# triq-org/spectroplot-js

Hardware: NVIDIA B200
Metric: Msamples/s rendered to RGBA spectrogram (N=4096) and % of B200 HBM roofline (higher is better)
Workload: dtype f32

## Files before the change

spectroplot-js_b200/csrc/sp_kernel_r64.cuh:

```cuda
#pragma once
#include "sp_prims.cuh"

#ifndef SP_XP
#define SP_XP 0
#endif
#ifndef SP_R64_TMA
#define SP_R64_TMA 1
#endif

namespace sp {

template <int FMT, bool SUB> struct R64Cfg {
    static constexpr int N = 4096, T = 64, STREAMS = 4, FFT_THREADS = T * STREAMS, STORE_THREADS = 128, THREADS = FFT_THREADS + STORE_THREADS;
    static constexpr int STEPS = 4, F = STREAMS * STEPS;
    static constexpr int FFT_REGS = 232, STORE_REGS = 40;
    static constexpr int SWB = SUB ? 8 : sample_width(FMT == FMT_RUNTIME ? CF64 : FMT);
    static constexpr bool OK = SUB || ((FMT != FMT_RUNTIME) && SWB <= 8);
    static constexpr int XP = 66;
    static constexpr int X_BYTES = 64 * XP * 8;
    static constexpr int WIN_PITCH = 64;
    static constexpr int TW_PITCH = 14;
    static constexpr int ST_PITCH = 1026;
    static constexpr int RING = 4;
    static constexpr bool TMA = SP_R64_TMA != 0;
    static constexpr int TILE_BYTES = TMA ? (STORE_THREADS / 32) * 4096 : 0;
    static constexpr size_t SMEM_BYTES = (size_t)STREAMS * X_BYTES + (size_t)F * ST_PITCH * 4 + (size_t)JH_SIZE * 4
                                       + ((SUB || TMA) ? 0 : (size_t)T * WIN_PITCH * 4) + TILE_BYTES + (size_t)T * TW_PITCH * 8 + 1024
                                       + (size_t)F * 2 * 8  + (size_t)2 * F * 8  + 192 + 1024 ;
    static_assert(SMEM_BYTES <= 232448, "render_r64_kernel: dynamic shared memory above the 227 KB an sm_100 CTA may have");
};

__device__ __forceinline__ unsigned lut_at(unsigned lut_base, unsigned word, int j)
{
    const unsigned a = ((j == 0 ? word << 2 : word >> (8 * j - 2)) & 0x3fcu) | lut_base;
    unsigned v;
    asm volatile("ld.shared.u32 %0, [%1];" : "=r"(v) : "r"(a));
    return v;
}

__device__ __forceinline__ void store_row8(uint32_t *rowp, uint4 a, uint4 b, bool aligned)
{
    if (aligned) st_global_256(rowp, a, b);
    else {
        rowp[0] = a.x; rowp[1] = a.y; rowp[2] = a.z; rowp[3] = a.w;
        rowp[4] = b.x; rowp[5] = b.y; rowp[6] = b.z; rowp[7] = b.w;
    }
}

__device__ __forceinline__ void stream_barrier(int stream)
{
    asm volatile("bar.sync %0, 64;" ::"r"(stream + 1) : "memory");
}

template <int FMT, bool SUB, bool OPT = false>
__global__ void __launch_bounds__(384, 1) render_r64_kernel(const Params p, const float2 *__restrict__ tw14, const __grid_constant__ CUtensorMap tmap)
{
    using B = R64Cfg<FMT, SUB>;
    constexpr int N = B::N, T = B::T, F = B::F;
    constexpr bool FLOAT_IN = SUB || FMT == CF32 || FMT == CF64 || FMT == FMT_RUNTIME;
    extern __shared__ __align__(128) unsigned char smem_r64[];
    const unsigned lut_base = (smem_u32(smem_r64) + 1023u) & ~1023u;
    unsigned char *s_x = smem_r64 + (lut_base - smem_u32(smem_r64)) + 1024;
    unsigned *s_lut = reinterpret_cast<unsigned *>(s_x - 1024);
    unsigned char *s_tiles = s_x + B::STREAMS * B::X_BYTES;
    unsigned *s_stage = reinterpret_cast<unsigned *>(s_tiles + B::TILE_BYTES);
    unsigned *s_jh = s_stage + F * B::ST_PITCH;
    float *s_win = reinterpret_cast<float *>(s_jh + JH_SIZE);
    float2 *s_tw = reinterpret_cast<float2 *>(s_win + ((SUB || B::TMA) ? 0 : T * B::WIN_PITCH));
    uint2 *s_mm = reinterpret_cast<uint2 *>(s_tw + T * B::TW_PITCH);
    float2 *s_fmid = reinterpret_cast<float2 *>(s_mm + F * 2);
    uint64_t *s_mbar = reinterpret_cast<uint64_t *>(s_fmid + 2 * F);
    int *s_off = reinterpret_cast<int *>(s_mbar + B::STREAMS);
    uint64_t *s_full = reinterpret_cast<uint64_t *>(s_off + B::STREAMS * 2);
    uint64_t *s_empty = s_full + 2;
    uint64_t *s_tready = s_empty + 2;
    long long *s_ring = reinterpret_cast<long long *>(s_tready + B::RING);
    long long *s_tile0 = s_ring + B::RING;

    const int tid = threadIdx.x;
    const int s = tid >> 6;
    const int t = tid & 63;
    float2 *X = reinterpret_cast<float2 *>(s_x + (size_t)s * B::X_BYTES);
    unsigned char *raw = reinterpret_cast<unsigned char *>(X);
    uint64_t *mbar = s_mbar + s;

    for (int i = tid; i < JH_SIZE; i += B::THREADS) s_jh[i] = 0;
    const int cmax = p.cmap_len - 1;
    const JhConst jc = jh_const(p);
    for (int i = tid; i < 256; i += B::THREADS) s_lut[i] = i <= cmax ? p.lut[jc.rev ? cmax - i : i] : 0u;
    for (int i = tid; i < T * B::TW_PITCH; i += B::THREADS) s_tw[i] = tw14[i];
    if constexpr (!SUB && !B::TMA)
        for (int i = tid; i < N; i += B::THREADS) s_win[(i & 63) * B::WIN_PITCH + (((i >> 6) + 4 * (i & 63)) & 63)] = p.window[i];
    const unsigned jh_base = smem_u32(s_jh) - (JH_MAGIC_BITS << 2);
    const int nfull = p.n_full, sub_r = p.sub_r;

    auto stage = [&](long long xr, int k0sub, unsigned par) {
        if (xr >= p.chunk_frames) xr = p.chunk_frames - 1;
        const void *src;
        unsigned bytes;
        if constexpr (SUB) {
            src = p.sub_in + ((size_t)xr * sub_r + (size_t)k0sub) * N;
            bytes = N * 8;
            s_off[s * 2 + par] = 0;
        } else {
            const long long xgl = p.frame_first + p.chunk_first + xr;
            const long long p0 = (long long)__dadd_rn(0.5, __dmul_rn(p.stride, (double)xgl)) - p.sample_base;
            const unsigned long long off = (unsigned long long)p0 * B::SWB, a0 = off & ~15ull;
            src = p.buf + a0;
            bytes = (unsigned)(((off - a0) + (unsigned long long)N * B::SWB + 15) & ~15ull);
            s_off[s * 2 + par] = (int)(off - a0);
        }
        tma_load_1d(raw, src, bytes, mbar);
    };
    auto tile_xr0 = [&](long long tile) -> long long { return (SUB ? tile / sub_r : tile) * F; };

    auto ticket = [&]() -> long long {
        const unsigned long long k = atomicAdd(p.tile_ctr, 1ull);
        if (k == (unsigned long long)p.ntiles + gridDim.x - 1) atomicExch(p.tile_ctr, 0ull);
        return (long long)k;
    };
    auto ring_put = [&](unsigned j, long long tl) {
        s_ring[(j - 1) % B::RING] = tl;
        mbar_arrive(s_tready + (j - 1) % B::RING);
    };
    auto ring_get = [&](unsigned j) -> long long {
        mbar_wait(s_tready + (j - 1) % B::RING, ((j - 1) / B::RING) & 1);
        return s_ring[(j - 1) % B::RING];
    };

    if (p.t_stamp && blockIdx.x == 0 && tid == 0) p.t_stamp[0] = globaltimer_ns();
    if (t == 0 && tid < B::FFT_THREADS) mbar_init(mbar, 1);
    if (tid == 0) {
        for (int h = 0; h < 2; h++) { mbar_init(s_full + h, B::FFT_THREADS / 32); mbar_init(s_empty + h, B::STORE_THREADS / 32); }
        for (int r = 0; r < B::RING; r++) mbar_init(s_tready + r, 1);
    }
    if (tid == B::FFT_THREADS) *s_tile0 = ticket();
    if (t == 0) asm volatile("fence.mbarrier_init.release.cluster;" ::: "memory");
    __syncthreads();
    long long tile = *s_tile0;
    unsigned kk = 0;

    if (tid >= B::FFT_THREADS) {
        asm volatile("setmaxnreg.dec.sync.aligned.u32 %0;" ::"n"(B::STORE_REGS));
        const int ht = tid - B::FFT_THREADS;
        const bool rows_aligned = (p.nframes % 8 == 0) && ((reinterpret_cast<uintptr_t>(p.image) & 31) == 0);
        if (ht == 0 && tile < p.ntiles) ring_put(1, ticket());
        griddep_wait();
        griddep_launch_dependents();
        while (tile < p.ntiles) {
            const int k0sub = SUB ? (int)(tile % sub_r) : 0;
            const long long xr0 = tile_xr0(tile);
#pragma unroll 1
            for (int h = 0; h < 2; h++) {
                mbar_wait(s_full + h, kk & 1);
                const size_t x0 = (size_t)(p.chunk_first + xr0) + 8 * h;
                const bool live = xr0 + 8 * h < p.chunk_frames;
                if constexpr (OPT && !SUB) {
                    if (p.waterfall && live) {
#pragma unroll 1
                        for (int f = 0; f < 8; f++) {
                            uint32_t *rowp = reinterpret_cast<uint32_t *>(p.image) + (size_t)N * (size_t)(p.nframes - 1 - (long long)(x0 + f));
                            const unsigned *src = s_stage + (8 * h + f) * B::ST_PITCH + ht;
#pragma unroll
                            for (int i = 0; i < 8; i++) {
                                const int id = ht + B::STORE_THREADS * i, k0 = id & 63, m = id >> 6;
                                const unsigned w = src[B::STORE_THREADS * i];
#pragma unroll
                                for (int j = 0; j < 4; j++)
                                    rowp[(k0 + 64 * (4 * m + j) + N / 2 - 1) & (N - 1)] = lut_at(lut_base, w, j);
                            }
                        }
                    }
                }
                if constexpr (B::TMA && !SUB) {
                    if (p.use_tma && live && (!OPT || !p.waterfall)) {
                        const int lane = ht & 31, wq = ht >> 5;
                        unsigned char *tile = s_tiles + wq * 4096;
                        const int r = 31 - lane;
                        const unsigned toff = (unsigned)(r * 32 + (((r >> 2) & 1) << 4));
#pragma unroll 1
                        for (int i = 0; i < 8; i++) {
                            const int id = ht + B::STORE_THREADS * i, k0 = id & 63, m = id >> 6;
                            const unsigned *src = s_stage + (8 * h) * B::ST_PITCH + m * 64 + k0;
                            unsigned w[8];
#pragma unroll
                            for (int f = 0; f < 8; f++) w[f] = src[f * B::ST_PITCH];
                            if (lane == 0) bulk_wait_read0();
                            __syncwarp();
#pragma unroll
                            for (int j = 0; j < 4; j++) {
                                uint4 a, b;
                                a.x = lut_at(lut_base, w[0], j); a.y = lut_at(lut_base, w[1], j); a.z = lut_at(lut_base, w[2], j); a.w = lut_at(lut_base, w[3], j);
                                b.x = lut_at(lut_base, w[4], j); b.y = lut_at(lut_base, w[5], j); b.z = lut_at(lut_base, w[6], j); b.w = lut_at(lut_base, w[7], j);
                                *reinterpret_cast<uint4 *>(tile + j * 1024 + toff) = a;
                                *reinterpret_cast<uint4 *>(tile + j * 1024 + (toff ^ 16u)) = b;
                                if (k0 + 64 * (4 * m + j) == N / 2)
                                    st_global_256(reinterpret_cast<uint32_t *>(p.image) + x0, a, b);
                            }
                            fence_async_smem();
                            __syncwarp();
                            if (lane == 0) {
                                const int kb0 = (k0 & 32) + 256 * m;
#pragma unroll
                                for (int j = 0; j < 4; j++)
                                    tma_store_2d(&tmap, smem_u32(tile + j * 1024), (int)x0, (N / 2 - (kb0 + 64 * j) - 31) & (N - 1));
                                bulk_commit();
                            }
                        }
                    }
                }
#pragma unroll 1
                for (int i = 0; i < ((live && (!OPT || SUB || !p.waterfall) && !(B::TMA && !SUB && p.use_tma)) ? 8 : 0); i++) {
                    const int id = ht + B::STORE_THREADS * i, k0 = id & 63, m = id >> 6;
                    const unsigned *src = s_stage + (8 * h) * B::ST_PITCH + m * 64 + k0;
                    unsigned w[8];
#pragma unroll
                    for (int f = 0; f < 8; f++) w[f] = src[f * B::ST_PITCH];
#pragma unroll
                    for (int j = 0; j < 4; j++) {
                        const int kb = k0 + 64 * (4 * m + j);
                        const int bin = SUB ? k0sub + sub_r * kb : kb;
                        const int y = (nfull / 2 - bin) & (nfull - 1);
                        uint32_t *rowp = reinterpret_cast<uint32_t *>(p.image) + (size_t)p.nframes * (size_t)y + x0;
                        uint4 a, b;
                        if (!(p.dbg & 4)) {
                            a.x = lut_at(lut_base, w[0], j); a.y = lut_at(lut_base, w[1], j); a.z = lut_at(lut_base, w[2], j); a.w = lut_at(lut_base, w[3], j);
                            b.x = lut_at(lut_base, w[4], j); b.y = lut_at(lut_base, w[5], j); b.z = lut_at(lut_base, w[6], j); b.w = lut_at(lut_base, w[7], j);
                        } else { a = make_uint4(w[0], w[1], w[2], w[3]); b = make_uint4(w[4], w[5], w[6], w[7]); }
                        if (!(p.dbg & 1)) store_row8(rowp, a, b, rows_aligned);
                    }
                }
                if (ht < 8 && live) {
                    const int fl = 8 * h + ht;
                    const long long xl = p.chunk_first + xr0 + fl;
                    const uint2 m0 = s_mm[fl * 2], m1 = s_mm[fl * 2 + 1];
                    const unsigned umn = min(m0.x, m1.x), umx = max(m0.y, m1.y);
                    const float mn = fminf(0.0f, fmaf(fast_log2(__uint_as_float(umn)), p.c1, p.c0));
                    const float mx = fmaxf(-200.0f, fmaf(fast_log2(__uint_as_float(umx)), p.c1, p.c0));
                    if constexpr (SUB) {
                        atomicMin(reinterpret_cast<unsigned *>(p.fmin) + xl, f2ord(mn));
                        atomicMax(reinterpret_cast<unsigned *>(p.fmax) + xl, f2ord(mx));
                    } else { p.fmin[xl] = mn; p.fmax[xl] = mx; p.fmid[xl] = s_fmid[(kk & 1) * F + fl]; }
                }
                __syncwarp();
                if ((ht & 31) == 0) mbar_arrive(s_empty + h);
            }
            tile = ring_get(++kk);
            if (ht == 0 && tile < p.ntiles) ring_put(kk + 1, ticket());
        }
        if constexpr (B::TMA && !SUB) bulk_wait_read0();
    } else {
    asm volatile("setmaxnreg.inc.sync.aligned.u32 %0;" ::"n"(B::FFT_REGS));
    unsigned fpar = 0;
    if (t == 0 && tile < p.ntiles) stage(tile_xr0(tile) + s, SUB ? (int)(tile % sub_r) : 0, 0);

    while (tile < p.ntiles) {
        const int k0sub = SUB ? (int)(tile % sub_r) : 0;
        const long long xr0 = tile_xr0(tile);
        long long next_tile = 0;

#pragma unroll 1
        for (int step = 0; step < B::STEPS; step++) {
            const int fl = step * B::STREAMS + s;
            const bool valid = xr0 + fl < p.chunk_frames;
            const unsigned jbase = valid ? jh_base : jh_base + (smem_u32(s_stage + 8 * B::ST_PITCH) - smem_u32(s_jh));
            int half = step >> 1;
            asm volatile("" : "+r"(half));
            if (step == B::STEPS - 1) next_tile = ring_get(kk + 1);
            cf v[64];
            const bool split = OPT && !SUB && p.channel_mode;
            auto prefetch = [&]() {
                if (step < B::STEPS - 1) stage(xr0 + fl + B::STREAMS, k0sub, fpar);
                else if (next_tile < p.ntiles) stage(tile_xr0(next_tile) + s, SUB ? (int)(next_tile % sub_r) : 0, fpar);
            };
            mbar_wait(mbar, fpar);
            if constexpr (SUB) {
#pragma unroll
                for (int n0 = 0; n0 < 8; n0++)
#pragma unroll
                    for (int n1 = 0; n1 < 8; n1++) v[8 * n1 + n0] = cld(reinterpret_cast<const float2 *>(raw) + T * (8 * n1 + n0) + t);
            } else {
                const unsigned char *rp = raw + s_off[s * 2 + fpar];
                const float4 *wrow = B::TMA ? p.window_t + t : reinterpret_cast<const float4 *>(s_win + t * B::WIN_PITCH);
#pragma unroll
                for (int qq = 0; qq < 16; qq++) {
                    const int q = 2 * (qq & 7) + (qq >> 3);
                    const float4 w = (SP_XP & 4) ? make_float4(1.f, 1.f, 1.f, 1.f) : B::TMA ? __ldg(wrow + 64 * q) : wrow[(q + t) & 15];
                    cf d[4];
#pragma unroll
                    for (int c = 0; c < 4; c++) d[c] = decode_raw_cf<FMT>(rp, T * (4 * q + c) + t, p.format);
                    if (q == 8 && t == 0 && valid) s_fmid[(kk & 1) * F + fl] = make_float2(cre(d[0]) * raw_scale<FMT>(), cim(d[0]) * raw_scale<FMT>());
                    v[4 * q] = cscale(d[0], w.x);     v[4 * q + 1] = cscale(d[1], w.y);
                    v[4 * q + 2] = cscale(d[2], w.z); v[4 * q + 3] = cscale(d[3], w.w);
                }
            }
            fpar ^= 1;
            dft64_between(v, [&] { stream_barrier(s); });
            {
                const float4 *twp = reinterpret_cast<const float4 *>(s_tw + t * B::TW_PITCH);
                float2 w[8];
                const float4 a = twp[0], b = twp[1], c = twp[2], d = twp[3];
                w[1] = make_float2(a.x, a.y); w[2] = make_float2(a.z, a.w); w[3] = make_float2(b.x, b.y); w[4] = make_float2(b.z, b.w);
                w[5] = make_float2(c.x, c.y); w[6] = make_float2(c.z, c.w); w[7] = make_float2(d.x, d.y);
#pragma unroll
                for (int j = 1; j < 8; j++) v[j] = cmul(v[j], w[j]);
#pragma unroll
                for (int j = 0; j < 8; j++) cst(X + j * B::XP + t, v[j]);
                float2 hi[8];
                hi[1] = make_float2(d.z, d.w);
                const float4 e = twp[4], f = twp[5], g = twp[6];
                hi[2] = make_float2(e.x, e.y); hi[3] = make_float2(e.z, e.w); hi[4] = make_float2(f.x, f.y);
                hi[5] = make_float2(f.z, f.w); hi[6] = make_float2(g.x, g.y); hi[7] = make_float2(g.z, g.w);
#pragma unroll
                for (int i = 1; i < 8; i++) {
                    v[8 * i] = cmul(v[8 * i], hi[i]);
#pragma unroll
                    for (int j = 1; j < 8; j++) v[8 * i + j] = cmul(v[8 * i + j], (SP_XP & 8) ? w[j] : cun(cmul(cpk(hi[i]), w[j])));
#pragma unroll
                    for (int j = 0; j < 8; j++) cst(X + (8 * i + j) * B::XP + t, v[8 * i + j]);
                }
            }
            stream_barrier(s);
            {
                const float4 *row = reinterpret_cast<const float4 *>(X + t * B::XP);
#pragma unroll
                for (int mm = 0; mm < 32; mm++) {
                    const int m = 4 * (mm & 7) + (mm >> 3);
                    const float4 q = row[m];
                    v[2 * m] = cpk(q.x, q.y); v[2 * m + 1] = cpk(q.z, q.w);
                }
            }
            dft64_between(v, [&] {
                stream_barrier(s);
                if (t == 0 && !split) prefetch();
            });
            if ((step & 1) == 0) mbar_wait(s_empty + half, (kk + 1) & 1);
            {
                {
                    if constexpr (OPT && !SUB) {
                        if (split) {
                            auto split_lo = [](cf a, cf b) {
                                const float2 fb = cun(b);
                                return cscale(cadd(a, cpk(fb.x, -fb.y)), 0.5f);
                            };
                            auto split_hi = [](cf a, cf b) {
                                const float2 fa = cun(a), fb = cun(b);
                                return cscale(cadd(cpk(fa.y, fa.x), cpk(fb.y, -fb.x)), 0.5f);
                            };
                            {
                                float4 *wrow = reinterpret_cast<float4 *>(X + t * B::XP);
#pragma unroll
                                for (int m = 0; m < 32; m++) {
                                    const float2 a = cun(v[2 * m]), b = cun(v[2 * m + 1]);
                                    wrow[m] = make_float4(a.x, a.y, b.x, b.y);
                                }
                            }
                            stream_barrier(s);
                            if (t == 0) {
#pragma unroll
                                for (int k1 = 1; k1 < 32; k1++) {
                                    const cf a = v[k1], b = v[64 - k1];
                                    v[k1] = split_lo(a, b);
                                    v[64 - k1] = split_hi(b, a);
                                }
                                v[0] = cpk(fmaf(0.0f, cim(v[0]), cre(v[0])), 0.0f);
                                v[32] = cpk(0.0f, 0.0f);
                            } else {
                                const float4 *prow = reinterpret_cast<const float4 *>(X + (64 - t) * B::XP);
#pragma unroll
                                for (int a = 0; a < 32; a++) {
                                    const float4 q = prow[31 - a];
                                    if (a < 16) {
                                        v[2 * a] = split_lo(v[2 * a], cpk(q.z, q.w));
                                        v[2 * a + 1] = split_lo(v[2 * a + 1], cpk(q.x, q.y));
                                    } else {
                                        v[2 * a] = split_hi(v[2 * a], cpk(q.z, q.w));
                                        v[2 * a + 1] = split_hi(v[2 * a + 1], cpk(q.x, q.y));
                                    }
                                }
                            }
                            stream_barrier(s);
                            if (t == 0) prefetch();
                        }
                    }

                    float amin = __int_as_float(0x7f800000), amax = 0.0f, prev = 0.0f;
                    unsigned umin_i = 0x7f800000u, umax_i = 0u;
                    unsigned *stg = s_stage + fl * B::ST_PITCH + t;
#pragma unroll
                    for (int m = 0; m < 16; m++) {
                        unsigned yb[4];
#pragma unroll
                        for (int j = 0; j < 4; j++) {
                            const float2 vi = cun(v[4 * m + j]);
                            const float abs2 = fmaf(vi.x, vi.x, vi.y * vi.y);
                            if constexpr (FLOAT_IN) {
                                umin_i = min(umin_i, __float_as_uint(abs2));
                                umax_i = max(umax_i, __float_as_uint(abs2));
                            } else if (j & 1) {
                                amin = fmin3(amin, prev, abs2);
                                amax = fmax3(amax, prev, abs2);
                            } else prev = abs2;
                            const float l2 = (SP_XP & 16) ? abs2 : fast_log2(abs2);
                            float Y;
                            const float S = (SP_XP & 16) ? (Y = l2, __uint_as_float((__float_as_uint(l2) >> 20) + JH_MAGIC_BITS)) : jh_eval(l2, jc, Y);
                            if constexpr ((SP_XP & 1) != 0) red_shared_inc_addr(smem_u32(s_jh) + ((tid & 31) << 2) + (__float_as_uint(S) & 0x380u));
                            else if constexpr (!(SP_XP & 2)) red_shared_inc_addr(jbase + (__float_as_uint(S) << 2));
                            yb[j] = __float_as_uint(Y);
                        }
                        stg[m * 64] = __byte_perm(__byte_perm(yb[0], yb[1], 0x0040), __byte_perm(yb[2], yb[3], 0x0040), 0x5410);
                    }
                    unsigned umn, umx;
                    if constexpr (FLOAT_IN) {
                        umn = __reduce_min_sync(0xffffffffu, umin_i);
                        umx = __reduce_max_sync(0xffffffffu, umax_i);
                    } else {
                        umn = __reduce_min_sync(0xffffffffu, __float_as_uint(amin));
                        umx = __reduce_max_sync(0xffffffffu, __float_as_uint(amax));
                    }
                    if (umn < 0x00800000u || umx >= 0x7f800000u) {
                        unsigned nzero = 0, nbad = 0, nnan = 0;
                        float mn = __int_as_float(0x7f800000), mx = 0.0f;
#pragma unroll
                        for (int i = 0; i < 64; i++) {
                            const float2 vi = cun(v[i]);
                            const float abs2 = fmaf(vi.x, vi.x, vi.y * vi.y);
                            nzero += abs2 < 1.17549435e-38f ? 1u : 0u;
                            nbad += !(abs2 <= 3.402823466e38f) ? 1u : 0u;
                            nnan += abs2 != abs2 ? 1u : 0u;
                            mn = fminf(mn, abs2 < 1.17549435e-38f ? 0.0f : abs2);
                            mx = fmaxf(mx, abs2);
                        }
                        nzero = __reduce_add_sync(0xffffffffu, nzero);
                        nbad = __reduce_add_sync(0xffffffffu, nbad);
                        nnan = __reduce_add_sync(0xffffffffu, nnan);
                        umn = __reduce_min_sync(0xffffffffu, __float_as_uint(mn));
                        umx = __reduce_max_sync(0xffffffffu, __float_as_uint(mx));
                        if ((t & 31) == 0 && valid) {
                            if (nzero) atomicAdd(&s_jh[JH_ZERO], nzero);
                            if (nbad) atomicAdd(&s_jh[JH_BAD], nbad);
                            if (nnan) {
                                float Yn;
                                const float Sn = jh_eval(__int_as_float(0x7fffffff), jc, Yn);
                                atomicSub(&s_jh[__float_as_uint(Sn) - JH_MAGIC_BITS], nnan);
                                atomicAdd(&s_jh[JH_NAN], nnan);
                            }
                        }
                    }
                    if ((t & 31) == 0) s_mm[fl * 2 + (t >> 5)] = make_uint2(umn, umx);
                    if (step & 1) {
                        __syncwarp();
                        if ((t & 31) == 0) mbar_arrive(s_full + half);
                    }
                }
            }
        }
        tile = next_tile;
        kk++;
    }
    }

    __syncthreads();
    griddep_wait();
    for (int i = tid; i < JH_SIZE; i += B::THREADS)
        if (s_jh[i]) atomicAdd(&p.j_hist[i], (unsigned long long)s_jh[i]);
}

}
```

spectroplot-js_b200/csrc/sp_prims.cuh:

```cuda
#pragma once
#include "sp_kernels.cuh"
#include <cuda.h>

namespace sp {

__device__ __forceinline__ uint32_t smem_u32(const void *p) { return (uint32_t)__cvta_generic_to_shared(p); }

__device__ __forceinline__ void mbar_init(uint64_t *bar, unsigned count)
{
    asm volatile("mbarrier.init.shared::cta.b64 [%0], %1;" ::"r"(smem_u32(bar)), "r"(count));
}
__device__ __forceinline__ void mbar_wait(uint64_t *bar, unsigned parity)
{
    asm volatile(
        "{\n\t.reg .pred p;\n\t"
        "WAIT_%=:\n\t"
        "mbarrier.try_wait.parity.shared::cta.b64 p, [%0], %1;\n\t"
        "@p bra DONE_%=;\n\t"
        "bra WAIT_%=;\n\t"
        "DONE_%=:\n\t}" ::"r"(smem_u32(bar)), "r"(parity) : "memory");
}
__device__ __forceinline__ void mbar_arrive(uint64_t *bar)
{
    asm volatile("mbarrier.arrive.shared::cta.b64 _, [%0];" ::"r"(smem_u32(bar)) : "memory");
}
__device__ __forceinline__ void tma_load_1d(void *dst_smem, const void *src_gmem, unsigned bytes, uint64_t *bar)
{
    asm volatile("fence.proxy.async.shared::cta;" ::: "memory");
    asm volatile("mbarrier.arrive.expect_tx.shared::cta.b64 _, [%0], %1;" ::"r"(smem_u32(bar)), "r"(bytes) : "memory");
    asm volatile("cp.async.bulk.shared::cluster.global.mbarrier::complete_tx::bytes [%0], [%1], %2, [%3];"
                 ::"r"(smem_u32(dst_smem)), "l"(src_gmem), "r"(bytes), "r"(smem_u32(bar)) : "memory");
}
__device__ __forceinline__ void st_global_256(void *p, uint4 a, uint4 b)
{
    asm volatile("st.global.v8.b32 [%0], {%1, %2, %3, %4, %5, %6, %7, %8};" ::"l"(p), "r"(a.x), "r"(a.y), "r"(a.z), "r"(a.w),
                 "r"(b.x), "r"(b.y), "r"(b.z), "r"(b.w) : "memory");
}
__device__ __forceinline__ void red_shared_inc(unsigned *p)
{
    asm volatile("red.shared.add.u32 [%0], 1;" ::"r"(smem_u32(p)) : "memory");
}

__device__ __forceinline__ void red_shared_inc_addr(unsigned addr)
{
    asm volatile("red.shared.add.u32 [%0], 1;" ::"r"(addr) : "memory");
}


__device__ __forceinline__ void tma_store_2d(const void *tmap, unsigned smem_src, int x, int y)
{
    asm volatile("cp.async.bulk.tensor.2d.global.shared::cta.bulk_group [%0, {%2, %3}], [%1];"
                 ::"l"(tmap), "r"(smem_src), "r"(x), "r"(y) : "memory");
}
__device__ __forceinline__ void bulk_commit() { asm volatile("cp.async.bulk.commit_group;" ::: "memory"); }
__device__ __forceinline__ void bulk_wait_read0() { asm volatile("cp.async.bulk.wait_group.read 0;" ::: "memory"); }
__device__ __forceinline__ void fence_async_smem() { asm volatile("fence.proxy.async.shared::cta;" ::: "memory"); }

}
```

Measured before the change: 423,500.

## Hold twiddles and window coefficients in tensor memory instead of smem and L1

Allocates 256 TMEM columns per CTA and has two FFT warpgroups precompute the full per-lane twiddle table (including the products of the high and low twiddles) and the transposed window into it at kernel start. Inside the DFT loop the FFT threads fetch these with double-buffered tcgen05.ld rather than reading shared memory, recomputing twiddle products with complex multiplies, or issuing __ldg of the window per sample group. The aim is to take shared-memory bandwidth and arithmetic off the FFT path and shrink the smem footprint. In exchange it adds TMEM allocation, fences and a named barrier, plus load latency that the double buffering has to hide.

```diff
diff --git a/spectroplot-js_b200/csrc/sp_kernel_r64.cuh b/spectroplot-js_b200/csrc/sp_kernel_r64.cuh
--- a/spectroplot-js_b200/csrc/sp_kernel_r64.cuh
+++ b/spectroplot-js_b200/csrc/sp_kernel_r64.cuh
@@ -18,14 +18,13 @@
     static constexpr bool OK = SUB || ((FMT != FMT_RUNTIME) && SWB <= 8);
     static constexpr int XP = 66;
     static constexpr int X_BYTES = 64 * XP * 8;
-    static constexpr int WIN_PITCH = 64;
-    static constexpr int TW_PITCH = 14;
+    static constexpr int TMEM_COLS = 256, WIN_COL = 128;
     static constexpr int ST_PITCH = 1026;
     static constexpr int RING = 4;
     static constexpr bool TMA = SP_R64_TMA != 0;
     static constexpr int TILE_BYTES = TMA ? (STORE_THREADS / 32) * 4096 : 0;
     static constexpr size_t SMEM_BYTES = (size_t)STREAMS * X_BYTES + (size_t)F * ST_PITCH * 4 + (size_t)JH_SIZE * 4
-                                       + ((SUB || TMA) ? 0 : (size_t)T * WIN_PITCH * 4) + TILE_BYTES + (size_t)T * TW_PITCH * 8 + 1024
+                                       + TILE_BYTES + 1024
                                        + (size_t)F * 2 * 8  + (size_t)2 * F * 8  + 192 + 1024 ;
     static_assert(SMEM_BYTES <= 232448, "render_r64_kernel: dynamic shared memory above the 227 KB an sm_100 CTA may have");
 };
@@ -65,9 +64,7 @@
     unsigned char *s_tiles = s_x + B::STREAMS * B::X_BYTES;
     unsigned *s_stage = reinterpret_cast<unsigned *>(s_tiles + B::TILE_BYTES);
     unsigned *s_jh = s_stage + F * B::ST_PITCH;
-    float *s_win = reinterpret_cast<float *>(s_jh + JH_SIZE);
-    float2 *s_tw = reinterpret_cast<float2 *>(s_win + ((SUB || B::TMA) ? 0 : T * B::WIN_PITCH));
-    uint2 *s_mm = reinterpret_cast<uint2 *>(s_tw + T * B::TW_PITCH);
+    uint2 *s_mm = reinterpret_cast<uint2 *>(s_jh + JH_SIZE);
     float2 *s_fmid = reinterpret_cast<float2 *>(s_mm + F * 2);
     uint64_t *s_mbar = reinterpret_cast<uint64_t *>(s_fmid + 2 * F);
     int *s_off = reinterpret_cast<int *>(s_mbar + B::STREAMS);
@@ -76,8 +73,10 @@
     uint64_t *s_tready = s_empty + 2;
     long long *s_ring = reinterpret_cast<long long *>(s_tready + B::RING);
     long long *s_tile0 = s_ring + B::RING;
+    uint32_t *s_tmem = reinterpret_cast<uint32_t *>(s_tile0 + 1);
 
     const int tid = threadIdx.x;
+    if (tid < 32) tmem_alloc(s_tmem, B::TMEM_COLS);
     const int s = tid >> 6;
     const int t = tid & 63;
     float2 *X = reinterpret_cast<float2 *>(s_x + (size_t)s * B::X_BYTES);
@@ -88,9 +87,6 @@
     const int cmax = p.cmap_len - 1;
     const JhConst jc = jh_const(p);
     for (int i = tid; i < 256; i += B::THREADS) s_lut[i] = i <= cmax ? p.lut[jc.rev ? cmax - i : i] : 0u;
-    for (int i = tid; i < T * B::TW_PITCH; i += B::THREADS) s_tw[i] = tw14[i];
-    if constexpr (!SUB && !B::TMA)
-        for (int i = tid; i < N; i += B::THREADS) s_win[(i & 63) * B::WIN_PITCH + (((i >> 6) + 4 * (i & 63)) & 63)] = p.window[i];
     const unsigned jh_base = smem_u32(s_jh) - (JH_MAGIC_BITS << 2);
     const int nfull = p.n_full, sub_r = p.sub_r;
 
@@ -136,7 +132,9 @@
     }
     if (tid == B::FFT_THREADS) *s_tile0 = ticket();
     if (t == 0) asm volatile("fence.mbarrier_init.release.cluster;" ::: "memory");
+    tmem_fence_before_sync();
     __syncthreads();
+    tmem_fence_after_sync();
     long long tile = *s_tile0;
     unsigned kk = 0;
 
@@ -253,6 +251,42 @@
     asm volatile("setmaxnreg.inc.sync.aligned.u32 %0;" ::"n"(B::FFT_REGS));
     unsigned fpar = 0;
     if (t == 0 && tile < p.ntiles) stage(tile_xr0(tile) + s, SUB ? (int)(tile % sub_r) : 0, 0);
+    const uint32_t tm = *s_tmem + ((uint32_t)(32 * ((tid >> 5) & 3)) << 16);
+    if (s < 2) {
+        const float2 *tr = tw14 + t * 14;
+        float2 w[8];
+#pragma unroll
+        for (int j = 1; j < 8; j++) w[j] = tr[j - 1];
+#pragma unroll 1
+        for (int i = 0; i < 8; i++) {
+            const float2 hi = i == 0 ? make_float2(1.0f, 0.0f) : tr[6 + i];
+            uint32_t r[16];
+#pragma unroll
+            for (int j = 0; j < 8; j++) {
+                const float2 x = j == 0 ? hi : i == 0 ? w[j] : cun(cmul(cpk(hi), w[j]));
+                r[2 * j] = __float_as_uint(x.x); r[2 * j + 1] = __float_as_uint(x.y);
+            }
+            tmem_st16(tm + 16 * i, r);
+        }
+        if constexpr (!SUB) {
+#pragma unroll 1
+            for (int g = 0; g < 4; g++) {
+                uint32_t r[16];
+#pragma unroll
+                for (int u = 0; u < 4; u++) {
+                    const int qq = 4 * g + u, q = 2 * (qq & 7) + (qq >> 3);
+                    const float4 c = p.window_t[64 * q + t];
+                    r[4 * u] = __float_as_uint(c.x); r[4 * u + 1] = __float_as_uint(c.y);
+                    r[4 * u + 2] = __float_as_uint(c.z); r[4 * u + 3] = __float_as_uint(c.w);
+                }
+                tmem_st16(tm + B::WIN_COL + 16 * g, r);
+            }
+        }
+        tmem_wait_st();
+    }
+    tmem_fence_before_sync();
+    asm volatile("bar.sync 5, %0;" ::"n"(B::FFT_THREADS) : "memory");
+    tmem_fence_after_sync();
 
     while (tile < p.ntiles) {
         const int k0sub = SUB ? (int)(tile % sub_r) : 0;
@@ -273,6 +307,8 @@
                 if (step < B::STEPS - 1) stage(xr0 + fl + B::STREAMS, k0sub, fpar);
                 else if (next_tile < p.ntiles) stage(tile_xr0(next_tile) + s, SUB ? (int)(next_tile % sub_r) : 0, fpar);
             };
+            [[maybe_unused]] uint32_t wq[2][16];
+            if (!SUB && !(SP_XP & 4)) tmem_ld16(tm + B::WIN_COL, wq[0]);
             mbar_wait(mbar, fpar);
             if constexpr (SUB) {
 #pragma unroll
@@ -281,11 +317,16 @@
                     for (int n1 = 0; n1 < 8; n1++) v[8 * n1 + n0] = cld(reinterpret_cast<const float2 *>(raw) + T * (8 * n1 + n0) + t);
             } else {
                 const unsigned char *rp = raw + s_off[s * 2 + fpar];
-                const float4 *wrow = B::TMA ? p.window_t + t : reinterpret_cast<const float4 *>(s_win + t * B::WIN_PITCH);
 #pragma unroll
                 for (int qq = 0; qq < 16; qq++) {
                     const int q = 2 * (qq & 7) + (qq >> 3);
-                    const float4 w = (SP_XP & 4) ? make_float4(1.f, 1.f, 1.f, 1.f) : B::TMA ? __ldg(wrow + 64 * q) : wrow[(q + t) & 15];
+                    if (!(SP_XP & 4) && (qq & 3) == 0) {
+                        tmem_wait_ld(wq[(qq >> 2) & 1]);
+                        if (qq < 12) tmem_ld16(tm + B::WIN_COL + 4 * (qq + 4), wq[((qq >> 2) + 1) & 1]);
+                    }
+                    const uint32_t *wr = wq[(qq >> 2) & 1] + 4 * (qq & 3);
+                    const float4 w = (SP_XP & 4) ? make_float4(1.f, 1.f, 1.f, 1.f)
+                                                 : make_float4(__uint_as_float(wr[0]), __uint_as_float(wr[1]), __uint_as_float(wr[2]), __uint_as_float(wr[3]));
                     cf d[4];
 #pragma unroll
                     for (int c = 0; c < 4; c++) d[c] = decode_raw_cf<FMT>(rp, T * (4 * q + c) + t, p.format);
@@ -297,25 +338,21 @@
             fpar ^= 1;
             dft64_between(v, [&] { stream_barrier(s); });
             {
-                const float4 *twp = reinterpret_cast<const float4 *>(s_tw + t * B::TW_PITCH);
+                uint32_t tr[2][16];
                 float2 w[8];
-                const float4 a = twp[0], b = twp[1], c = twp[2], d = twp[3];
-                w[1] = make_float2(a.x, a.y); w[2] = make_float2(a.z, a.w); w[3] = make_float2(b.x, b.y); w[4] = make_float2(b.z, b.w);
-                w[5] = make_float2(c.x, c.y); w[6] = make_float2(c.z, c.w); w[7] = make_float2(d.x, d.y);
-#pragma unroll
-                for (int j = 1; j < 8; j++) v[j] = cmul(v[j], w[j]);
-#pragma unroll
-                for (int j = 0; j < 8; j++) cst(X + j * B::XP + t, v[j]);
-                float2 hi[8];
-                hi[1] = make_float2(d.z, d.w);
-                const float4 e = twp[4], f = twp[5], g = twp[6];
-                hi[2] = make_float2(e.x, e.y); hi[3] = make_float2(e.z, e.w); hi[4] = make_float2(f.x, f.y);
-                hi[5] = make_float2(f.z, f.w); hi[6] = make_float2(g.x, g.y); hi[7] = make_float2(g.z, g.w);
-#pragma unroll
-                for (int i = 1; i < 8; i++) {
-                    v[8 * i] = cmul(v[8 * i], hi[i]);
-#pragma unroll
-                    for (int j = 1; j < 8; j++) v[8 * i + j] = cmul(v[8 * i + j], (SP_XP & 8) ? w[j] : cun(cmul(cpk(hi[i]), w[j])));
+                tmem_ld16(tm, tr[0]);
+#pragma unroll
+                for (int i = 0; i < 8; i++) {
+                    tmem_wait_ld(tr[i & 1]);
+                    if (i < 7) tmem_ld16(tm + 16 * (i + 1), tr[(i + 1) & 1]);
+                    const uint32_t *r = tr[i & 1];
+                    auto tw = [&](int j) { return make_float2(__uint_as_float(r[2 * j]), __uint_as_float(r[2 * j + 1])); };
+                    if (i == 0) {
+#pragma unroll
+                        for (int j = 1; j < 8; j++) w[j] = tw(j);
+                    } else v[8 * i] = cmul(v[8 * i], tw(0));
+#pragma unroll
+                    for (int j = 1; j < 8; j++) v[8 * i + j] = cmul(v[8 * i + j], (SP_XP & 32) && i > 0 ? cun(cmul(cpk(tw(0)), w[j])) : tw(j));
 #pragma unroll
                     for (int j = 0; j < 8; j++) cst(X + (8 * i + j) * B::XP + t, v[8 * i + j]);
                 }
@@ -458,6 +495,12 @@
         tile = next_tile;
         kk++;
     }
+    tmem_fence_before_sync();
+    asm volatile("bar.sync 5, %0;" ::"n"(B::FFT_THREADS) : "memory");
+    if (tid < 32) {
+        tmem_fence_after_sync();
+        tmem_dealloc(tm, B::TMEM_COLS);
+    }
     }
 
     __syncthreads();
diff --git a/spectroplot-js_b200/csrc/sp_prims.cuh b/spectroplot-js_b200/csrc/sp_prims.cuh
--- a/spectroplot-js_b200/csrc/sp_prims.cuh
+++ b/spectroplot-js_b200/csrc/sp_prims.cuh
@@ -56,4 +56,36 @@
 __device__ __forceinline__ void bulk_wait_read0() { asm volatile("cp.async.bulk.wait_group.read 0;" ::: "memory"); }
 __device__ __forceinline__ void fence_async_smem() { asm volatile("fence.proxy.async.shared::cta;" ::: "memory"); }
 
+__device__ __forceinline__ void tmem_alloc(uint32_t *dst_smem, unsigned ncols)
+{
+    asm volatile("tcgen05.alloc.cta_group::1.sync.aligned.shared::cta.b32 [%0], %1;" ::"r"(smem_u32(dst_smem)), "r"(ncols) : "memory");
+    asm volatile("tcgen05.relinquish_alloc_permit.cta_group::1.sync.aligned;" ::: "memory");
 }
+__device__ __forceinline__ void tmem_dealloc(uint32_t taddr, unsigned ncols)
+{
+    asm volatile("tcgen05.dealloc.cta_group::1.sync.aligned.b32 %0, %1;" ::"r"(taddr), "r"(ncols) : "memory");
+}
+__device__ __forceinline__ void tmem_fence_before_sync() { asm volatile("tcgen05.fence::before_thread_sync;" ::: "memory"); }
+__device__ __forceinline__ void tmem_fence_after_sync() { asm volatile("tcgen05.fence::after_thread_sync;" ::: "memory"); }
+__device__ __forceinline__ void tmem_ld16(uint32_t taddr, uint32_t (&r)[16])
+{
+    asm volatile("tcgen05.ld.sync.aligned.32x32b.x16.b32 {%0,%1,%2,%3,%4,%5,%6,%7,%8,%9,%10,%11,%12,%13,%14,%15}, [%16];"
+                 : "=r"(r[0]), "=r"(r[1]), "=r"(r[2]), "=r"(r[3]), "=r"(r[4]), "=r"(r[5]), "=r"(r[6]), "=r"(r[7]),
+                   "=r"(r[8]), "=r"(r[9]), "=r"(r[10]), "=r"(r[11]), "=r"(r[12]), "=r"(r[13]), "=r"(r[14]), "=r"(r[15])
+                 : "r"(taddr));
+}
+__device__ __forceinline__ void tmem_wait_ld(uint32_t (&r)[16])
+{
+    asm volatile("tcgen05.wait::ld.sync.aligned;"
+                 : "+r"(r[0]), "+r"(r[1]), "+r"(r[2]), "+r"(r[3]), "+r"(r[4]), "+r"(r[5]), "+r"(r[6]), "+r"(r[7]),
+                   "+r"(r[8]), "+r"(r[9]), "+r"(r[10]), "+r"(r[11]), "+r"(r[12]), "+r"(r[13]), "+r"(r[14]), "+r"(r[15]));
+}
+__device__ __forceinline__ void tmem_st16(uint32_t taddr, const uint32_t (&r)[16])
+{
+    asm volatile("tcgen05.st.sync.aligned.32x32b.x16.b32 [%0], {%1,%2,%3,%4,%5,%6,%7,%8,%9,%10,%11,%12,%13,%14,%15,%16};"
+                 ::"r"(taddr), "r"(r[0]), "r"(r[1]), "r"(r[2]), "r"(r[3]), "r"(r[4]), "r"(r[5]), "r"(r[6]), "r"(r[7]),
+                   "r"(r[8]), "r"(r[9]), "r"(r[10]), "r"(r[11]), "r"(r[12]), "r"(r[13]), "r"(r[14]), "r"(r[15]) : "memory");
+}
+__device__ __forceinline__ void tmem_wait_st() { asm volatile("tcgen05.wait::st.sync.aligned;" ::: "memory"); }
+
+}
```

Result: no change. 424,800 (median of 6 runs) (+0.3%).
